# camillabelponer/dealii-slod

Hardware: AMD Instinct MI355X
Metric: SLOD patches/sec (basis built), 2D Poisson H=1/32 n_sub=8 oversampling 2 (higher is better)
Workload: dtype f64; 1 GPU; C2: 2D Poisson SLOD, H=1/32, n_sub=8, oversampling=2, D1e4 coefficient (contrast 10000), 1024 patches on rank 0 (ensemble of 1 realisations, contiguous patch blocks); patches_per_gpu=1024, parallelism=patch-sharded x1

## Files before the change

### dealii-slod_amd/csrc/slod_api.cpp

```cpp
#include "slod_host.h"

#include <algorithm>
#include <cmath>
#include <cstdio>
#include <cstdlib>
#include <cstring>
#include <string>
#include <vector>

namespace
{
  struct PatchGeom
  {
    int cx, cy, x0, y0, mx, my;
    int side_domain[4];
  };
}

std::string &slod_create_error()
{
  static thread_local std::string e;
  return e;
}

// ... 151 lines not shown
  {
    const slod_handle *h = p->h;
    SlodKernelArgs     a;
    std::memset(&a, 0, sizeof(a));
    a.desc        = (balanced && p->d_desc_bal ? p->d_desc_bal : p->d_desc) + first;
    a.coef0       = h->d_coef[0];
    a.coef1       = h->d_coef[1];
    a.coef_stride = (size_t)h->NE * h->NE * 4;
    a.NE          = h->NE;
    a.n_sub       = h->cfg.n_subdivisions;
    a.quirk       = h->cfg.projection_quirk;
#ifdef SLOD_ENABLE_DIAG
    if (const char *dg = std::getenv("SLOD_DIAG"))
      a.diag = std::atoi(dg);
#endif
    const double H = 1.0 / (double)h->N, hh = H / (double)h->cfg.n_subdivisions;
    a.scale     = hh * hh / 4.0;
    a.invH2     = 1.0 / (H * H);
    a.st        = p->ws_st;
    a.st_stride = p->st_stride;
    a.nn_max    = p->nn_max;
    a.vinv      = p->ws_v;
    a.v_stride  = p->v_stride;
    a.m_max     = p->m_max;
    a.L_max     = p->L_max;
    a.xs        = p->ws_x;
    a.zs        = p->ws_z ? p->ws_z : p->ws_x;
    a.x_stride  = p->x_stride;
    a.nc_max    = p->nc_max;
    a.ms        = p->ws_m;
    a.mt        = p->ws_m + p->chunk * (size_t)p->nc_max * p->nc_max;
    a.m_fused   = 0;
    a.m_tw      = 0;
    a.nb_buf    = p->nb_buf;
    a.nf_max    = p->nf_max;
    a.fuse_select = 0;
    a.fuse_assemble = 0;
    a.basis     = d_basis;
    a.premult   = d_premult;
    a.status    = p->d_status;
    a.pdiag     = p->d_pdiag;
    if (slot == 1)
      {
        a.st     = p->alt.ws_st;
        a.vinv   = p->alt.ws_v;
        a.xs     = p->alt.ws_x;
        a.zs     = p->alt.ws_z ? p->alt.ws_z : p->alt.ws_x;
        a.ms     = p->alt.ws_m;
        a.mt     = p->alt.ws_m + p->chunk * (size_t)p->nc_max * p->nc_max;
        a.status = p->alt.d_status;
      }
    return a;
  }
}

namespace
{
  hipError_t launch_range(slod_plan *p, size_t first, int cnt, double *d_basis, double *d_premult, hipStream_t st,
                          hipEvent_t *ev, bool balanced, int slot = 0)
  {
    const int      s = p->h->cfg.spacedim;
    SlodKernelArgs a = make_args(p, first, d_basis, d_premult, balanced, slot);
    hipError_t     e = ev ? hipEventRecord(ev[0], st) : hipSuccess;
    if (e == hipSuccess && !p->choice.fuse_assemble)
      e = slod_launch_assemble(s, a, cnt, st);
    if (e == hipSuccess && ev)
// ... 1013 lines not shown
```

### dealii-slod_amd/csrc/slod_device.h

```cpp
#ifndef SLOD_DEVICE_H
#define SLOD_DEVICE_H

#include <hip/hip_runtime.h>
#include <stddef.h>
#include <stdint.h>

struct SlodPatchDesc
{
  int32_t  ox, oy;
  int32_t  nx, ny;
  int32_t  mx, my;
  int32_t  ccx, ccy;
  int32_t  flags;
  int32_t  m, L;
  int32_t  n_c, n_b;
  int32_t  prob;
  uint32_t plan_index;
  uint64_t out_off;
};

__host__ __device__ inline size_t slod_mt_stride(int nc_max) { return (size_t)nc_max * nc_max + 1; }

enum : int32_t
{
// ... 16 lines not shown
  double  dinf;
  double  sigma_max, sigma_min;
};

struct SlodKernelArgs
{
  const SlodPatchDesc *desc;
  const double        *coef0;
  const double        *coef1;
  size_t               coef_stride;
  int32_t              NE;
  int32_t              n_sub;
  int32_t              quirk;
  int32_t              diag;
  int32_t              debug;
  double               scale;
  double               invH2;
  double *st;
  size_t  st_stride;
  int32_t nn_max;
  double *vinv;
  size_t  v_stride;
  int32_t m_max;
  int32_t L_max;
  int32_t nv;
  double *xs;
  double *zs;
  size_t  x_stride;
  int32_t nc_max;
  double *ms;
  int32_t m_fused;
  double *mt;
  int32_t m_tw;
  int32_t nb_buf;
  int32_t nf_max;
  int32_t fuse_select;
  int32_t fuse_assemble;
  double  *basis;
  double  *premult;
  int32_t *status;
  SlodPatchDiag *pdiag;
};

enum SlodSolverKind : int32_t
{
  SLOD_K_MF   = 1,
  SLOD_K_TW   = 2,
  SLOD_K_WS   = 3,
  SLOD_K_COOP = 4,
  SLOD_K_ND   = 5
};

struct SlodTuning
{
  int solver = 0;
  int fuse_select = 1, fuse_assemble = 1, fuse_m = -1;
  int twisted = -1;
  int balance = 1;
  int debug = 0;
};
struct SlodSolveChoice
{
  int    kind = 0;
  size_t lds  = 0;
  int    fuse_select = 0, fuse_assemble = 0, m_fused = 0, m_tw = 0, twisted = 0, debug = 0;
  int    v_line_pad = 0;
  size_t v_line_elems = 0;
  int    nv = 0;
  size_t v_patch_elems = 0;
};
SlodTuning slod_read_tuning();
bool       slod_choose_solver(int S, int n_sub, int m_max, int L_max, int nc_max, int nb_buf, int nf_max, size_t n_patches,
                              const SlodTuning &t, SlodSolveChoice *out);

hipError_t slod_launch_assemble(int S, const SlodKernelArgs &a, int n_patches, hipStream_t st);
hipError_t slod_launch_solve(int S, const SlodSolveChoice &c, SlodKernelArgs &a, int n_patches, hipStream_t st);
hipError_t slod_launch_solve_mf(int S, const SlodKernelArgs &a, int n_patches, size_t lds, hipStream_t st);
hipError_t slod_launch_solve_tw(int S, const SlodKernelArgs &a, int n_patches, size_t lds, hipStream_t st);
hipError_t slod_launch_solve_ws(int S, const SlodKernelArgs &a, int n_patches, size_t lds, hipStream_t st);
hipError_t slod_launch_solve_coop(int S, int twisted, const SlodKernelArgs &a, int n_patches, hipStream_t st);
hipError_t slod_launch_solve_nd(const SlodKernelArgs &a, int n_patches, size_t lds, hipStream_t st);
int        slod_solve_nd_cell(int S, int n_sub, int m_max, int L_max);
size_t     slod_solve_nd_scratch(int nv, int m_max, int L_max, int nc_max);
size_t     slod_solve_nd_lds_bytes(int nv, int m_max, int nc_max);
hipError_t slod_launch_select(int S, const SlodKernelArgs &a, int n_patches, int nb_max,
                              int nf_max, hipStream_t st);
size_t     slod_solve_lds_bytes(int S, int m_max, int nc_max, int twisted);
size_t     slod_solve_ws_lds_bytes(int S, int m_max, int nc_max);
size_t     slod_solve_tw_lds_bytes(int S, int m_max, int nc_max, bool with_m = false);
size_t     slod_solve_mf_lds_bytes(int S, int m_max, int nc_max);
int        slod_solve_ws_tile(int m_max);
int        slod_solve_mf_tiles(int S, int m_max);
size_t     slod_select_lds_bytes(int S, int nb_max, int nc_max, int nf_max);

#endif
```

### dealii-slod_amd/csrc/slod_dispatch.cpp

```cpp
#include "slod_device.h"

#include <algorithm>
#include <cstdlib>
#include <cstring>

SlodTuning slod_read_tuning()
{
  SlodTuning t;
  if (const char *sel = getenv("SLOD_SOLVE"))
    t.solver = !strcmp(sel, "mf") ? SLOD_K_MF : !strcmp(sel, "tw") ? SLOD_K_TW : !strcmp(sel, "ws") ? SLOD_K_WS :
               !strcmp(sel, "coop") ? SLOD_K_COOP : !strcmp(sel, "nd") ? SLOD_K_ND : 0;
  if (const char *e = getenv("SLOD_FUSE_SELECT"))
    t.fuse_select = atoi(e) ? 1 : 0;
  if (const char *e = getenv("SLOD_FUSE_ASSEMBLE"))
    t.fuse_assemble = atoi(e) ? 1 : 0;
  if (const char *e = getenv("SLOD_FUSE_M"))
    t.fuse_m = atoi(e) ? 1 : 0;
  if (const char *e = getenv("SLOD_TWISTED"))
    t.twisted = atoi(e) ? 1 : 0;
  if (const char *e = getenv("SLOD_BALANCE"))
    t.balance = atoi(e) ? 1 : 0;
  if (const char *e = getenv("SLOD_DEBUG"))
    t.debug = atoi(e) ? 1 : 0;
  return t;
}

bool slod_choose_solver(int S, int n_sub, int m_max, int L_max, int nc_max, int nb_buf, int nf_max, size_t n_patches,
                        const SlodTuning &t_in, SlodSolveChoice *out)
{
  const size_t    lds_max = 160 * 1024;
  SlodSolveChoice c;
  const int       nd_nv = slod_solve_nd_cell(S, n_sub, m_max, L_max);
  SlodTuning      t     = t_in;
  if (t.solver == SLOD_K_ND && nd_nv == 0)
    t.solver = 0;
  c.debug = t.debug;
  const int  wt = slod_solve_ws_tile(m_max);
  const bool ws_fits = wt > 0 && wt >= 2 * S - 1;
  const auto want = [&](int k) { return t.solver == 0 || t.solver == k; };
  const size_t lds_sel = slod_select_lds_bytes(S, nb_buf, nc_max, nf_max);
  const bool   mf_fits = slod_solve_mf_tiles(S, m_max) > 0 && slod_solve_mf_lds_bytes(S, m_max, nc_max) <= lds_max;
  const bool   tw_fits = ws_fits && slod_solve_tw_lds_bytes(S, m_max, nc_max) <= lds_max;
  if (nd_nv > 0 && t.solver == SLOD_K_ND)
    {
      c.kind          = SLOD_K_ND;
      c.nv            = nd_nv;
      c.lds           = slod_solve_nd_lds_bytes(nd_nv, m_max, nc_max);
      c.v_patch_elems = slod_solve_nd_scratch(nd_nv, m_max, L_max, nc_max);
      c.fuse_assemble = t.fuse_assemble ? 1 : 0;
      c.fuse_select   = 0;
    }
  else if (mf_fits && (t.solver == SLOD_K_MF || (t.solver == 0 && !tw_fits && !ws_fits)))
    {
      c.kind          = SLOD_K_MF;
      c.lds           = slod_solve_mf_lds_bytes(S, m_max, nc_max);
      c.v_line_pad    = 16 * slod_solve_mf_tiles(S, m_max);
      c.v_line_elems  = (size_t)c.v_line_pad * c.v_line_pad;
      c.fuse_assemble = (S == 1 && t.fuse_assemble) ? 1 : 0;
      c.fuse_select   = (S == 1 && t.fuse_select && lds_sel <= lds_max) ? 1 : 0;
      if (c.fuse_select && lds_sel > c.lds)
        c.lds = lds_sel;
    }
  else if (want(SLOD_K_TW) && tw_fits)
    {
      c.kind          = SLOD_K_TW;
      c.lds           = slod_solve_tw_lds_bytes(S, m_max, nc_max);
      c.v_line_pad    = 8 * wt;
      c.v_line_elems  = (size_t)64 * wt * wt;
      c.fuse_assemble = (S == 1 && t.fuse_assemble) ? 1 : 0;
      c.fuse_select = (S == 1 && t.fuse_select && lds_sel <= 64 * 1024) ? 1 : 0;
      if (S == 1 && t.fuse_m != 0 && nc_max <= 32 && 8 * wt <= 48)
        {
          const size_t sel    = c.fuse_select ? lds_sel : 0;
          const size_t with_m = std::max(slod_solve_tw_lds_bytes(S, m_max, nc_max, true), sel);
          if (std::min<size_t>(4, lds_max / with_m) == std::min<size_t>(4, lds_max / std::max(c.lds, sel)))
            {
              c.m_tw = 1;
              c.lds  = slod_solve_tw_lds_bytes(S, m_max, nc_max, true);
            }
        }
      if (c.fuse_select && lds_sel > c.lds)
        c.lds = lds_sel;
    }
  else if ((want(SLOD_K_WS) || t.solver == SLOD_K_TW) && ws_fits &&
           slod_solve_ws_lds_bytes(S, m_max, nc_max) <= lds_max)
    {
      c.kind       = SLOD_K_WS;
      c.lds        = slod_solve_ws_lds_bytes(S, m_max, nc_max);
      c.v_line_pad = 8 * wt;
      c.v_line_elems = (size_t)c.v_line_pad * c.v_line_pad;
      c.m_fused = (t.fuse_m > 0 && nc_max * nc_max <= 192 * 4) ? 1 : 0;
    }
  else if (t.solver == 0 || t.solver == SLOD_K_COOP || !ws_fits)
    {
      int tw = t.twisted >= 0 ? t.twisted : (n_patches < 3 * 256 ? 1 : 0);
      if (slod_solve_lds_bytes(S, m_max, nc_max, tw) > lds_max)
        tw = 0;
      if (slod_solve_lds_bytes(S, m_max, nc_max, tw) > lds_max || (m_max + 15) / 16 > 7)
        return false;
      c.kind       = SLOD_K_COOP;
      c.twisted    = tw;
      c.lds        = slod_solve_lds_bytes(S, m_max, nc_max, tw);
      c.v_line_pad = m_max;
      c.v_line_elems = (size_t)m_max * m_max;
    }
  else
    return false;
  if (!c.fuse_select && lds_sel > lds_max)
    return false;
  *out = c;
  return true;
}

hipError_t slod_launch_solve(int S, const SlodSolveChoice &c, SlodKernelArgs &a, int n_patches, hipStream_t st)
{
  a.m_fused       = c.m_fused;
  a.m_tw          = c.m_tw;
  a.fuse_select   = c.fuse_select;
  a.fuse_assemble = c.fuse_assemble;
  a.debug         = c.debug;
  switch (c.kind)
    {
      case SLOD_K_MF:
        return slod_launch_solve_mf(S, a, n_patches, c.lds, st);
      case SLOD_K_TW:
        return slod_launch_solve_tw(S, a, n_patches, c.lds, st);
      case SLOD_K_WS:
        return slod_launch_solve_ws(S, a, n_patches, c.lds, st);
      case SLOD_K_COOP:
        return slod_launch_solve_coop(S, c.twisted, a, n_patches, st);
      case SLOD_K_ND:
        a.nv = c.nv;
        return slod_launch_solve_nd(a, n_patches, c.lds, st);
      default:
        return hipErrorInvalidValue;
    }
}
```

### dealii-slod_amd/csrc/slod_solve_tw.hip

```cpp
#include <type_traits>
#include "slod_assemble.hip.h"
#include "slod_select.hip.h"

namespace
{
  template <int T, int S>
  __global__ __launch_bounds__(256, ws_min_waves(T)) void k_solve_tw(const SlodKernelArgs A)
  {
    extern __shared__ __attribute__((aligned(16))) double smem[];
    const SlodPatchDesc d = A.desc[blockIdx.x];
    constexpr int       W = 2 * S - 1, BW = 2 * W + 1, MP = 8 * T;
    constexpr int       BWP = BW + 1, BROWS = MP + 2 * W, bsz = (BROWS * BWP + 1) & ~1;
    const int           tid = threadIdx.x, wave = __builtin_amdgcn_readfirstlane(tid >> 6);
    int                 lane = tid & 63;
    const int           chain = wave & 1;
    const bool          is_gj = wave < 2;
    const int           m = d.m, L = d.L, nc = d.n_c, n = A.n_sub;
    const int           mm = A.m_max, ncs = (A.nc_max + 1) & ~1, ncg = A.nc_max;
    const bool          tr  = (d.flags & SLOD_F_TRANSPOSED) != 0;
    const int           npx = d.nx + 1;
    const int           chsz = MP * ncs + MP + 6 * bsz;

    double *cb   = smem + chain * chsz;
    double *Rb   = cb;
    double *rowb = Rb + MP * ncs;
    double *Tf   = rowb + MP;
    double *Tn0  = Tf + bsz;
    double *Tn1  = Tn0 + bsz;
    double *Bc0  = Tn1 + bsz;
    double *Bc1  = Bc0 + bsz;
    auto    Bbuf = [&](double *base, int stp) { return base + ((stp + 3) % 3) * bsz; };
    double *ocb  = smem + (1 - chain) * chsz;
    int    *colk = reinterpret_cast<int *>(smem + 2 * chsz);
    int *perm = colk + 2 * A.nc_max + chain * 3 * A.nc_max, *inv = perm + A.nc_max, *act = inv + A.nc_max;
    int *operm = colk + 2 * A.nc_max + (1 - chain) * 3 * A.nc_max, *oinv = operm + A.nc_max, *oact = oinv + A.nc_max;
    (void)operm;
    double *mtile = smem + 2 * chsz + 4 * A.nc_max;
    double *mfull = smem + chsz;
    bool    mfuse = false;
    auto nafin = [&](int ch) {
      const int *ac = colk + 2 * A.nc_max + ch * 3 * A.nc_max + 2 * A.nc_max;
      const int  nl = ch == 0 ? L / 2 : L - 1 - L / 2;
      int        na = 0;
      for (int k = 0; k < nc; ++k)
        na += ac[k] <= nl - 1 ? 1 : 0;
      return na;
    };

    const double *st    = A.st + (size_t)blockIdx.x * A.st_stride;
    double       *vg    = A.vinv + (size_t)blockIdx.x * A.v_stride;
    double       *xg    = A.xs + (size_t)blockIdx.x * A.x_stride;
    double       *zg    = A.zs + (size_t)blockIdx.x * A.x_stride;
    const size_t  vline = (size_t)64 * T * T, xline = (size_t)mm * ncg;
    auto load_A = [&](const double *vl, int ti, double (&dst)[MP / 4]) __attribute__((always_inline)) {
      const int     row = min(16 * ti + (lane & 15), MP - 1);
      const int     rt = row / T, rr = row - rt * T, kq = lane >> 4;
      const double *base = vl + (rt * 8 + kq) * (T * T) + rr * T;
#pragma unroll
      for (int g = 0; g < 2; ++g)
#pragma unroll
        for (int kr = 0; kr < T; ++kr)
          dst[g * T + kr] = base[g * 4 * T * T + kr];
    };
    auto brow = [&](int kk) { return T * ((lane >> 4) + 4 * (kk / T)) + kk % T; };

    const int mid = L / 2;
    double4_t pm[3] = {{0.0, 0.0, 0.0, 0.0}, {0.0, 0.0, 0.0, 0.0}, {0.0, 0.0, 0.0, 0.0}};
    auto mid_tile = [&](int ti, bool with_m) __attribute__((always_inline)) {
      const double *vl = vg + (size_t)mid * vline;
      double       *xl = xg + (size_t)mid * xline;
      const int     tiles_j = (nc + 15) >> 4;
// ... 85 lines not shown
            }
          if (wave == nw - 1)
            turn(true);
        }
      __syncthreads();
    };
    const int n0 = mid, n1 = L - 1 - mid, nstp = n0 > n1 ? n0 : n1;
    const int nmy = chain == 0 ? n0 : n1;
    const int dl  = chain == 0 ? 1 : -1;
    auto      line_of = [&](int c, int t) { return c == 0 ? t : L - 1 - t; };

    if ((SLOD_DG(A, (1 << 20))) && tid == 0)
      {
        A.ms[(size_t)blockIdx.x * A.nc_max * A.nc_max] = (double)wall_clock64();
        if (A.nc_max * A.nc_max >= 16)
          {
            A.ms[(size_t)blockIdx.x * A.nc_max * A.nc_max + 12] = (double)__builtin_amdgcn_s_getreg((31 << 11) | 4);
            A.ms[(size_t)blockIdx.x * A.nc_max * A.nc_max + 13] = (double)__builtin_amdgcn_s_getreg((31 << 11) | 20);
          }
      }
    if ((SLOD_DG(A, (1 << 20))) && lane == 0 && A.nc_max * A.nc_max >= 24)
      A.ms[(size_t)blockIdx.x * A.nc_max * A.nc_max + 20 + wave] = (double)__builtin_amdgcn_s_getreg((31 << 11) | 4);
    auto tstamp = [&](int k) {
      if ((SLOD_DG(A, (1 << 20))) && tid == 0 && A.nc_max * A.nc_max >= 48)
        A.ms[(size_t)blockIdx.x * A.nc_max * A.nc_max + 32 + k] = (double)wall_clock64();
    };
    tstamp(0);
    if (S == 1 && A.fuse_assemble)
      {
        for (int node = tid; node < npx * (d.ny + 1); node += 256)
          assemble_node<S>(A, d, blockIdx.x, node);
        __syncthreads();
      }
    for (int idx = tid; idx < 2 * chsz; idx += 256)
      smem[idx] = 0.0;
    if (A.m_tw)
      for (int idx = tid; idx < 2 * 256; idx += 256)
        mtile[idx] = 0.0;
    for (int c = tid; c < nc; c += 256)
      {
        int kx, ky;
        cell_of_col(d, c / S, kx, ky);
        colk[c]            = kx;
        colk[A.nc_max + c] = ky;
      }
    __syncthreads();
    {
      auto first_step = [&](int ch, int c) {
        const int kq = tr ? colk[c] : colk[A.nc_max + c];
        const int a  = ch == 0 ? kq * n - 1 : L - (kq + 1) * n;
        return a > 0 ? a : 0;
      };
      for (int idx = tid; idx < 2 * nc; idx += 256)
        {
          const int ch = idx / nc, c = idx - ch * nc, a = first_step(ch, c);
          int       rank = 0;
          for (int c2 = 0; c2 < nc; ++c2)
            {
              const int a2 = first_step(ch, c2);
              rank += (a2 < a || (a2 == a && c2 < c)) ? 1 : 0;
            }
          int *pp = colk + 2 * A.nc_max + ch * 3 * A.nc_max;
          pp[rank]                = c;
          pp[A.nc_max + c]        = rank;
          pp[2 * A.nc_max + rank] = a;
        }
    }
    auto put_bands = [&](int line, double *Tdst, bool with_T, double *Bdst, int t0, int nt) __attribute__((always_inline)) {
      for (int idx = t0; idx < m * BW; idx += nt)
        {
          const int i = idx / BW, oi = idx - i * BW, o = oi - W;
          if (Tdst)
            Tdst[(i + W) * BWP + oi] = with_T ? coupling<S>(st, A.nn_max, npx, tr, m, line, i, 0, o) : 0.0;
          if (Bdst)
            Bdst[(i + W) * BWP + oi] = coupling<S>(st, A.nn_max, npx, tr, m, line, i, dl, o);
        }
    };
    auto put_step = [&](int stp, int t0, int nt) __attribute__((always_inline)) {
      if (stp >= nmy)
        return;
      put_bands(line_of(chain, stp + 1), (stp & 1) ? Tn1 : Tn0, !(chain == 1 && stp + 1 == nmy), nullptr, t0, nt);
      put_bands(line_of(chain, stp), nullptr, true, Bbuf(Bc0, stp), t0, nt);
    };
    {
      const int t0 = (wave >> 1) * 64 + lane;
      put_bands(line_of(chain, 0), Tf, true, nullptr, t0, 128);
      put_step(0, t0, 128);
      put_step(1, t0, 128);
    }
    __syncthreads();
    tstamp(1);
    mfuse = S == 1 && A.m_tw && (MP + 15) / 16 <= 3 && nc <= 32 &&
                 nc * nc <= MP * ncs + MP + 3 * bsz && !(SLOD_DG(A, 8));
    int na_end[2] = {0, 0};
    if (mfuse)
      {
        na_end[0] = __builtin_amdgcn_readfirstlane(nafin(0));
        na_end[1] = __builtin_amdgcn_readfirstlane(nafin(1));
        mfuse     = na_end[0] <= 16 && na_end[1] <= 16;
      }
    if (A.m_tw && tid == 0)
      A.mt[(size_t)blockIdx.x * slod_mt_stride(A.nc_max) + (size_t)A.nc_max * A.nc_max] = mfuse ? 1.0 : 0.0;

    if (is_gj)
      {
        __builtin_amdgcn_s_setprio(3);
        int    gy = lane >> 3, gx = lane & 7;
        double a[T][T];
        auto dpp_from_prev = [](double x) {
          const int lo = __builtin_amdgcn_update_dpp(0, __double2loint(x), 0x111, 0xf, 0xf, true);
          const int hi = __builtin_amdgcn_update_dpp(0, __double2hiint(x), 0x111, 0xf, 0xf, true);
          return __hiloint2double(hi, lo);
        };
        auto dpp_from_next = [](double x) {
          const int lo = __builtin_amdgcn_update_dpp(0, __double2loint(x), 0x101, 0xf, 0xf, true);
// ... 202 lines not shown
          for (int ta = 0; ta < T; ++ta)
#pragma unroll
            for (int tb = 0; tb < T; ++tb)
              tp[ta * T + tb] = sign * a[ta][tb];
        };
#pragma unroll
        for (int ta = 0; ta < T; ++ta)
#pragma unroll
          for (int tb = 0; tb < T; ++tb)
            {
              const int      i = T * gy + ta, j = T * gx + tb;
              const unsigned oi = (unsigned)(j - i + W);
              const double   v  = Tf[(i + W) * BWP + (oi < (unsigned)BW ? oi : (unsigned)BW)];
              a[ta][tb]         = (chain == 1 && nmy == 0) ? 0.0 : v;
            }
        double acc_t[4] = {0.0, 0.0, 0.0, 0.0};
        for (int t = 0; t < nstp; ++t)
          {
            const bool active = t < nmy;
            asm volatile("" : "+v"(lane));
            gy = lane >> 3;
            gx = lane & 7;
            const long long c0 = (SLOD_DG(A, (1 << 20))) ? wall_clock64() : 0;
            long long       c1 = c0, c2 = c0;
            if (active)
              {
                sweep();
                c1 = (SLOD_DG(A, (1 << 20))) ? wall_clock64() : 0;
                if (!(SLOD_DG(A, 32768)))
                  store_tile(vg + (size_t)line_of(chain, t) * vline, -1.0);
                if (SLOD_DG(A, (1 << 20)))
                  acc_t[3] += (double)(wall_clock64() - c1);
                if (!(SLOD_DG(A, 16384)))
                  next_S((t & 1) ? Tn1 : Tn0, Bbuf(Bc0, t));
                c2 = (SLOD_DG(A, (1 << 20))) ? wall_clock64() : 0;
              }
            __syncthreads();
            if (SLOD_DG(A, (1 << 20)))
              {
                const long long c3 = wall_clock64();
                acc_t[0] += (double)(c1 - c0);
                acc_t[1] += (double)(c2 - c1);
                acc_t[2] += (double)(c3 - c2);
              }
          }
        if ((SLOD_DG(A, (1 << 20))) && tid == 0 && A.nc_max * A.nc_max >= 48)
          {
            for (int k = 0; k < 4; ++k)
              A.ms[(size_t)blockIdx.x * A.nc_max * A.nc_max + 40 + k] = acc_t[k];
            if (A.nc_max * A.nc_max >= 52)
              for (int k = 0; k < 2; ++k)
                A.ms[(size_t)blockIdx.x * A.nc_max * A.nc_max + 48 + k] = acc_p[k];
          }
        tstamp(2);
        if (chain == 1)
          store_tile(vg + (size_t)mid * vline, 1.0);
        __syncthreads();
        if (chain == 0)
          {
            const double *w1 = vg + (size_t)mid * vline + (gy * 8 + gx) * (T * T);
#pragma unroll
            for (int ta = 0; ta < T; ++ta)
#pragma unroll
              for (int tb = 0; tb < T; ++tb)
                a[ta][tb] += w1[ta * T + tb];
            sweep();
            store_tile(vg + (size_t)mid * vline, -1.0);
// ... 162 lines not shown
                    {
                      acc0 = __builtin_amdgcn_mfma_f64_16x16x4f64(av[kk], bq[0][kk], acc0, 0, 0, 0);
                      if (two)
                        acc1 = __builtin_amdgcn_mfma_f64_16x16x4f64(av[kk], bq[1][kk], acc1, 0, 0, 0);
                    }
#pragma unroll
                  for (int r = 0; r < 4; ++r)
                    {
                      const int row = 16 * ti + (lane >> 4) + 4 * r, col = lane & 15;
                      if (row < m && col < ncols)
                        {
                          xl[row * ncols + col] = acc0[r];
                          Rb[row * ncs + col]   = acc0[r];
                        }
                      if (two && row < m && col + 16 < ncols)
                        {
                          xl[row * ncols + col + 16] = acc1[r];
                          Rb[row * ncs + col + 16]   = acc1[r];
                        }
                    }
                  if (ti + 1 < TI)
                    {
#pragma unroll
                      for (int kk = 0; kk < MP / 4; ++kk)
                        av[kk] = an[kk];
                    }
                }
            }
          __builtin_amdgcn_fence(__ATOMIC_RELEASE, "wavefront");
          __builtin_amdgcn_wave_barrier();
          if (mfuse)
            {
              __builtin_amdgcn_fence(__ATOMIC_ACQUIRE, "wavefront");
              double   *mtc = mtile + chain * 256 + (lane >> 4) * 16 + (lane & 15);
              double4_t macc;
#pragma unroll
              for (int r = 0; r < 4; ++r)
                macc[r] = mtc[64 * r];
#pragma unroll
              for (int kk = 0; kk < MP / 4; ++kk)
                macc = __builtin_amdgcn_mfma_f64_16x16x4f64(bq[0][kk], bp[brow(kk) * ncs], macc, 0, 0, 0);
#pragma unroll
              for (int r = 0; r < 4; ++r)
                mtc[64 * r] = macc[r];
              __builtin_amdgcn_fence(__ATOMIC_RELEASE, "wavefront");
              __builtin_amdgcn_wave_barrier();
            }
        };
        constexpr int NBQ = (MP * BW + 63) / 64;
        double        tq[NBQ], bq_[NBQ];
        auto fetch_step = [&](int stp) __attribute__((always_inline)) {
          const bool on = stp < nmy;
          const int  lT = line_of(chain, stp + 1), lB = line_of(chain, stp);
          const bool with_T = !(chain == 1 && stp + 1 == nmy);
#pragma unroll
          for (int q = 0; q < NBQ; ++q)
            {
              const int  idx = lane + 64 * q, i = idx / BW, oi = idx - i * BW, o = oi - W, j = i + o;
              const int  pi = i / S, ci = i - pi * S, pj = j / S, cj = j - pj * S, dp = pj - pi;
              const bool ok = on && idx < m * BW && j >= 0 && j < m && dp >= -1 && dp <= 1;
              const int ixT = tr ? lT + 1 : pi + 1, iyT = tr ? pi + 1 : lT + 1;
              const int ixB = tr ? lB + 1 : pi + 1, iyB = tr ? pi + 1 : lB + 1;
              const int dirT = (tr ? dp : 0) * 3 + (tr ? 0 : dp) + 4;
              const int dirB = ((tr ? dp : dl) + 1) * 3 + (tr ? dl : dp) + 1;
              const double vT = st[ok ? (size_t)((dirT * S + ci) * S + cj) * A.nn_max + ixT + iyT * npx : 0];
              const double vB = st[ok ? (size_t)((dirB * S + ci) * S + cj) * A.nn_max + ixB + iyB * npx : 0];
              tq[q]  = (ok && with_T) ? vT : 0.0;
              bq_[q] = ok ? vB : 0.0;
            }
        };
        auto store_step = [&](int stp) __attribute__((always_inline)) {
          if (stp >= nmy)
            return;
          double *Tdst = (stp & 1) ? Tn1 : Tn0, *Bdst = Bbuf(Bc0, stp);
#pragma unroll
          for (int q = 0; q < NBQ; ++q)
            {
              const int idx = lane + 64 * q, i = idx / BW, oi = idx - i * BW;
              if (idx < m * BW)
                {
                  Tdst[(i + W) * BWP + oi] = tq[q];
                  Bdst[(i + W) * BWP + oi] = bq_[q];
                }
            }
        };
        double acc_h[4] = {0.0, 0.0, 0.0, 0.0};
        int  na = 0;
        bool z_in_lds = false;
        auto fwd_step = [&](int tl) __attribute__((always_inline)) {
          const int na_prev = na;
          while (na < nc && act[na] <= tl)
            ++na;
          const int line = line_of(chain, tl);
          const long long b0 = (SLOD_DG(A, (1 << 20))) ? wall_clock64() : 0;
          const bool keep = TI <= 3 && na <= 32 && !(SLOD_DG(A, 8));
          if (keep)
            {
              double av[MP / 4];
              load_A(vg + (size_t)line * vline, 0, av);
              build_R(line, Bbuf(Bc0, tl - 1), tl > 0 ? zg + (size_t)line_of(chain, tl - 1) * xline : nullptr, na_prev,
                      true, false, na, perm, nullptr, act, tl - 1, z_in_lds);
              __builtin_amdgcn_fence(__ATOMIC_RELEASE, "wavefront");
              __builtin_amdgcn_wave_barrier();
              if (SLOD_DG(A, (1 << 20)))
                acc_h[3] += (double)(wall_clock64() - b0);
              gemm_Z_keep(line, na, zg + (size_t)line * xline, av);
              z_in_lds = true;
              return;
            }
          build_R(line, Bbuf(Bc0, tl - 1), tl > 0 ? zg + (size_t)line_of(chain, tl - 1) * xline : nullptr, na_prev, true,
                  false, na, perm, nullptr, act, tl - 1, false);
          __builtin_amdgcn_fence(__ATOMIC_RELEASE, "wavefront");
          __builtin_amdgcn_wave_barrier();
          if (SLOD_DG(A, (1 << 20)))
            acc_h[3] += (double)(wall_clock64() - b0);
          gemm_Z(line, na, zg + (size_t)line * xline, na);
          z_in_lds = false;
        };
        for (int t = 0; t < nstp; ++t)
          {
            asm volatile("" : "+v"(lane));
            const long long c0 = (SLOD_DG(A, (1 << 20))) ? wall_clock64() : 0;
            if (t > 0 && !(SLOD_DG(A, 32)))
              fetch_step(t + 1);
            if (t > 0 && t - 1 < nmy)
              fwd_step(t - 1);
            const long long c1 = (SLOD_DG(A, (1 << 20))) ? wall_clock64() : 0;
            if (t > 0 && !(SLOD_DG(A, 32)))
              store_step(t + 1);
            const long long c2 = (SLOD_DG(A, (1 << 20))) ? wall_clock64() : 0;
            __syncthreads();
            if (SLOD_DG(A, (1 << 20)))
              {
                const long long c3 = wall_clock64();
                acc_h[0] += (double)(c1 - c0);
                acc_h[1] += (double)(c2 - c1);
                acc_h[2] += (double)(c3 - c2);
              }
          }
        if ((SLOD_DG(A, (1 << 20))) && tid == 128 && A.nc_max * A.nc_max >= 48)
          for (int k = 0; k < 4; ++k)
            A.ms[(size_t)blockIdx.x * A.nc_max * A.nc_max + 44 + k] = acc_h[k];
        if (nmy == nstp && nmy > 0)
          fwd_step(nstp - 1);
        __syncthreads();
        if (chain == 0)
          {
            const double *B0 = Bbuf(Bc0, n0 - 1);
            double       *ob = ocb + MP * ncs + MP + 3 * bsz;
            const double *B1 = Bbuf(ob, n1 - 1);
            int na0 = 0, na1 = 0;
            while (na0 < nc && act[na0] <= n0 - 1)
              ++na0;
            while (na1 < nc && oact[na1] <= n1 - 1)
              ++na1;
            build_R(mid, B0, n0 > 0 ? zg + (size_t)(mid - 1) * xline : nullptr, na0, true, false, nc, nullptr, inv, act,
                    n0 - 1, false);
            __builtin_amdgcn_wave_barrier();
            if (n1 > 0)
              build_R(mid, B1, zg + (size_t)(mid + 1) * xline, na1, false, true, nc, nullptr, oinv, oact, n1 - 1, false);
            __builtin_amdgcn_fence(__ATOMIC_RELEASE, "wavefront");
            __builtin_amdgcn_wave_barrier();
          }
        else if (mfuse)
          {
            const int na0 = na_end[0], na1 = na_end[1];
            for (int idx = lane; idx < nc * nc; idx += 64)
              {
                const int a = idx / nc, b = idx - a * nc, lo = min(a, b), hi = max(a, b);
                double    v = 0.0;
#pragma unroll
                for (int ch = 0; ch < 2; ++ch)
                  {
                    const int *ci = colk + 2 * A.nc_max + ch * 3 * A.nc_max + A.nc_max;
                    const int  i0 = ci[lo], j0 = ci[hi];
                    if (i0 < (ch ? na1 : na0) && j0 < (ch ? na1 : na0))
                      v += mtile[ch * 256 + i0 * 16 + j0];
                  }
                mfull[idx] = v;
              }
          }
        __syncthreads();
        mid_phase();
      }

    tstamp(3);
    {
      const int t128 = (wave >> 1) * 64 + lane, w2 = wave >> 1;
      const int tiles_i = (m + 15) >> 4, tiles_j = (nc + 15) >> 4;
      constexpr int NBV = (MP * BW + 127) / 128;
      double        bv[NBV];
      auto fetch_B = [&](int line) __attribute__((always_inline)) {
#pragma unroll
        for (int q = 0; q < NBV; ++q)
          {
            const int idx = t128 + 128 * q, i = idx / BW, o = idx - i * BW - W;
            bv[q] = (idx < m * BW) ? coupling<S>(st, A.nn_max, npx, tr, m, line, i, dl, o) : 0.0;
          }
      };
      auto store_B = [&](double *Bdst) __attribute__((always_inline)) {
#pragma unroll
        for (int q = 0; q < NBV; ++q)
          {
            const int idx = t128 + 128 * q, i = idx / BW, oi = idx - i * BW;
            if (idx < m * BW)
              Bdst[(i + W) * BWP + oi] = bv[q];
          }
      };
      const int tstart = (SLOD_DG(A, 16)) ? -1 : nstp - 1;
      if (tstart >= 0 && tstart < nmy)
        {
          fetch_B(line_of(chain, tstart));
          store_B((tstart & 1) ? Bc1 : Bc0);
        }
      else if (nmy > 0 && tstart >= 0)
        {
          fetch_B(line_of(chain, nmy - 1));
          store_B(((nmy - 1) & 1) ? Bc1 : Bc0);
        }
      int nab = nc;
      constexpr int TIB   = (MP + 15) / 16;
      const bool    keepb = TIB <= 3 && nc <= 32 && !(SLOD_DG(A, 64));
      if (keepb)
        for (int idx = t128; idx < m * nc; idx += 128)
          {
            const int i = idx / nc, c = idx - i * nc;
            Rb[i * ncs + c] = xg[(size_t)mid * xline + i * ncg + c];
          }
      auto backward = [&](auto KEEP) __attribute__((always_inline)) {
      constexpr bool keep_x = decltype(KEEP)::value;
      for (int t = tstart; t >= 0; --t)
        {
          while (nab > 0 && act[nab - 1] > t)
            --nab;
          const bool    active = t < nmy;
          const int     line = line_of(chain, t), prev = line_of(chain, t + 1);
          const double *Bn = (t & 1) ? Bc1 : Bc0;
          asm volatile("" : "+v"(lane));
          __syncthreads();
          if (active && t > 0)
            fetch_B(line_of(chain, t - 1));
          if constexpr (keep_x)
            {
              const double *vl = vg + (size_t)line * vline;
              double       *xl = xg + (size_t)line * xline;
              const int     g = lane >> 3, cq = lane & 7;
              const int     colw = 16 * w2 + (lane & 15);
              const bool    gemm = active && 16 * w2 < nc;
              constexpr int NPRE = 1;
              double        av[NPRE][MP / 4], zl[NPRE][4];
              const double *zrow = zg + (size_t)line * xline;
              const int     zc   = colw < nc ? inv[colw] : nc;
              const bool    zok  = zc < nab;
              auto          load_Z = [&](int ti, double (&dst)[4]) __attribute__((always_inline)) {
#pragma unroll
                for (int r = 0; r < 4; ++r)
                  {
                    const int    row = 16 * ti + (lane >> 4) + 4 * r;
                    const bool   ok  = row < m && zok;
                    const double z   = zrow[ok ? row * nab + zc : 0];
                    dst[r]           = ok ? z : 0.0;
                  }
              };
              if (gemm)
                {
#pragma unroll
                  for (int ti = 0; ti < NPRE; ++ti)
                    if (ti < tiles_i)
                      {
                        load_A(vl, ti, av[ti]);
                        load_Z(ti, zl[ti]);
                      }
                }
              double y[2][T];
              if (active)
                {
#pragma unroll
                  for (int k = 0; k < 2; ++k)
                    {
                      const int c = cq + 8 * (2 * w2 + k);
                      double    win[T + 2 * W];
#pragma unroll
                      for (int e = 0; e < T + 2 * W; ++e)
                        {
                          const int    pr  = T * g + e - W;
                          const bool   inb = c < nc && pr >= 0 && pr < m;
                          const double x   = Rb[(inb ? pr : 0) * ncs + (inb ? c : 0)];
                          win[e]           = inb ? x : 0.0;
                        }
#pragma unroll
                      for (int ta = 0; ta < T; ++ta)
                        {
                          double v = 0.0;
#pragma unroll
                          for (int o = 0; o < BW; ++o)
                            v = fma(Bn[(T * g + ta + W) * BWP + o], win[ta + o], v);
                          y[k][ta] = v;
                        }
                    }
                }
              __builtin_amdgcn_fence(__ATOMIC_RELEASE, "wavefront");
              __builtin_amdgcn_wave_barrier();
              __builtin_amdgcn_fence(__ATOMIC_ACQUIRE, "wavefront");
              if (active)
                {
#pragma unroll
                  for (int k = 0; k < 2; ++k)
                    {
                      const int c = cq + 8 * (2 * w2 + k);
#pragma unroll
                      for (int ta = 0; ta < T; ++ta)
                        if (c < nc && T * g + ta < m)
                          Rb[(T * g + ta) * ncs + c] = y[k][ta];
                    }
                }
              __builtin_amdgcn_fence(__ATOMIC_RELEASE, "wavefront");
              __builtin_amdgcn_wave_barrier();
              __builtin_amdgcn_fence(__ATOMIC_ACQUIRE, "wavefront");
              double bq[MP / 4];
              if (gemm)
                {
#pragma unroll
                  for (int kk = 0; kk < MP / 4; ++kk)
                    bq[kk] = Rb[brow(kk) * ncs + colw];
                }
              __builtin_amdgcn_fence(__ATOMIC_RELEASE, "wavefront");
              __builtin_amdgcn_wave_barrier();
              __builtin_amdgcn_fence(__ATOMIC_ACQUIRE, "wavefront");
              if (gemm)
                {
#pragma unroll
                  for (int ti = 0; ti < TIB; ++ti)
                    if (ti < tiles_i)
                      {
                        double4_t acc = {0.0, 0.0, 0.0, 0.0};
                        double    zt[4];
                        if (ti < NPRE)
                          {
#pragma unroll
                            for (int kk = 0; kk < MP / 4; ++kk)
                              acc = __builtin_amdgcn_mfma_f64_16x16x4f64(av[ti < NPRE ? ti : 0][kk], bq[kk], acc, 0, 0, 0);
#pragma unroll
                            for (int r = 0; r < 4; ++r)
                              zt[r] = zl[ti < NPRE ? ti : 0][r];
                          }
                        else
                          {
                            double al[MP / 4];
                            load_A(vl, ti, al);
                            load_Z(ti, zt);
#pragma unroll
                            for (int kk = 0; kk < MP / 4; ++kk)
                              acc = __builtin_amdgcn_mfma_f64_16x16x4f64(al[kk], bq[kk], acc, 0, 0, 0);
                          }
#pragma unroll
                        for (int r = 0; r < 4; ++r)
                          {
                            const int row = 16 * ti + (lane >> 4) + 4 * r;
                            if (row < m && colw < nc)
                              {
                                const double x       = zt[r] - acc[r];
                                xl[row * ncg + colw] = x;
                                Rb[row * ncs + colw] = x;
                              }
                          }
                      }
                }
              if (active && t > 0)
                store_B(((t - 1) & 1) ? Bc1 : Bc0);
              continue;
            }
          if (active)
            {
              const double *xp = xg + (size_t)prev * xline;
              const int     qr = t128 >> 5, i_lo = (qr * m) >> 2, i_hi = ((qr + 1) * m) >> 2;
              for (int r = t128 & 31; r < nc; r += 32)
                {
                  double win[BW];
#pragma unroll
                  for (int e = 0; e < BW; ++e)
                    {
                      const int p = i_lo + e - W;
                      win[e]      = (p >= 0 && p < m) ? xp[p * ncg + r] : 0.0;
                    }
                  for (int i = i_lo; i < i_hi; ++i)
                    {
                      const int    pn    = i + 1 + W;
                      const double xnext = (pn < m) ? xp[pn * ncg + r] : 0.0;
                      double       v     = 0.0;
#pragma unroll
                      for (int o = 0; o < BW; ++o)
                        v = fma(Bn[(i + W) * BWP + o], win[o], v);
                      Rb[i * ncs + r] = v;
#pragma unroll
                      for (int e = 0; e + 1 < BW; ++e)
                        win[e] = win[e + 1];
                      win[BW - 1] = xnext;
                    }
                }
            }
          __syncthreads();
          if (active)
// ... 4 lines not shown
                {
                  const int ti = tt / tiles_j, tj = tt - ti * tiles_j;
                  const int col = 16 * tj + (lane & 15);
                  const double *zrow = zg + (size_t)line * xline;
                  const int     zc   = col < nc ? inv[col] : nc;
                  const bool    zok  = zc < nab;
                  double        zl[4];
#pragma unroll
                  for (int r = 0; r < 4; ++r)
                    {
                      const int row = 16 * ti + (lane >> 4) + 4 * r;
                      zl[r]         = (row < m && zok) ? zrow[row * nab + zc] : 0.0;
                    }
                  double4_t     acc = {0.0, 0.0, 0.0, 0.0};
                  const double *bp  = Rb + col;
                  double        av[MP / 4];
                  load_A(vl, ti, av);
#pragma unroll
                  for (int kk = 0; kk < MP / 4; ++kk)
                    acc = __builtin_amdgcn_mfma_f64_16x16x4f64(av[kk], bp[brow(kk) * ncs], acc, 0, 0, 0);
#pragma unroll
                  for (int r = 0; r < 4; ++r)
                    {
                      const int row = 16 * ti + (lane >> 4) + 4 * r;
                      if (row < m && col < nc)
                        xl[row * ncg + col] = zl[r] - acc[r];
                    }
                }
              if (t > 0)
                store_B(((t - 1) & 1) ? Bc1 : Bc0);
            }
        }
      };
      if (keepb)
        backward(std::true_type{});
      else
        backward(std::false_type{});
    }
    const bool stamp = (SLOD_DG(A, (1 << 20))) && tid == 0;
    if (stamp)
      A.ms[(size_t)blockIdx.x * A.nc_max * A.nc_max + 1] = (double)wall_clock64();
    if (S == 1 && A.fuse_select)
      {
        __syncthreads();
        select_patch<S>(A, A.nb_buf, A.nf_max, blockIdx.x, smem,
                        mfuse ? A.mt + (size_t)blockIdx.x * slod_mt_stride(A.nc_max) : nullptr);
        if (stamp)
          A.ms[(size_t)blockIdx.x * A.nc_max * A.nc_max + 2] = (double)wall_clock64();
      }
  }

}

size_t slod_solve_tw_lds_bytes(int S, int m_max, int nc_max, bool with_m)
{
  const int    T = slod_solve_ws_tile(m_max), W = 2 * S - 1, BW = 2 * W + 1, MP = 8 * T;
  const int    ncs = (nc_max + 1) & ~1, bsz = ((MP + 2 * W) * (BW + 1) + 1) & ~1;
  (void)m_max;
  const size_t chsz  = (size_t)MP * ncs + MP + 6 * (size_t)bsz;
  const size_t mtile = with_m ? 2 * 256 * sizeof(double) : 0;
  return ((2 * chsz * sizeof(double) + 8 * (size_t)nc_max * sizeof(int) + mtile) + 15) & ~(size_t)15;
}

template <int T, int S>
static hipError_t launch_tw_TS(const SlodKernelArgs &a, int n_patches, size_t lds, hipStream_t st)
{
  const void *fn = reinterpret_cast<const void *>(k_solve_tw<T, S>);
  hipError_t  e  = hipFuncSetAttribute(fn, hipFuncAttributeMaxDynamicSharedMemorySize, (int)lds);
  if (e != hipSuccess)
    return e;
  if (a.debug)
    {
      int nb = 0;
      (void)hipOccupancyMaxActiveBlocksPerMultiprocessor(&nb, fn, 256, lds);
      fprintf(stderr, "[slod] k_solve_tw<%d,%d>: %d patches, lds %zu B, occupancy %d blocks/CU, M in the sweeps %d\n", T,
              S, n_patches, lds, nb, a.m_tw);
    }
  hipLaunchKernelGGL((k_solve_tw<T, S>), dim3(n_patches), dim3(256), lds, st, a);
  return hipGetLastError();
}

template <int S>
static hipError_t launch_tw_S(const SlodKernelArgs &a, int n_patches, size_t lds, hipStream_t st)
{
  switch (slod_solve_ws_tile(a.m_max))
    {
      case 2:
        return launch_tw_TS<2, S>(a, n_patches, lds, st);
      case 3:
        return launch_tw_TS<3, S>(a, n_patches, lds, st);
      case 4:
        return launch_tw_TS<4, S>(a, n_patches, lds, st);
      case 5:
        return launch_tw_TS<5, S>(a, n_patches, lds, st);
      case 6:
        return launch_tw_TS<6, S>(a, n_patches, lds, st);
      case 8:
        return launch_tw_TS<8, S>(a, n_patches, lds, st);
      case 10:
        return launch_tw_TS<10, S>(a, n_patches, lds, st);
      case 12:
        return launch_tw_TS<12, S>(a, n_patches, lds, st);
      case 14:
        return launch_tw_TS<14, S>(a, n_patches, lds, st);
      default:
        return hipErrorInvalidValue;
    }
}

// ... 5 lines not shown
```

Before: 1.045 million patches/s.

## Stream backward-sweep V tiles into LDS via global_load_lds DMA in twisted solver

Adds an optional mode, on by default under SLOD_BW_DMA, for the twisted block-tridiagonal solver with S=1. In this mode the backward sweep copies the later V (inverse block) tiles of each line into LDS with global_load_lds direct-to-LDS transfers and reads the MFMA A operands from LDS instead of global memory. To fit this, the LDS layout is rearranged so the two chains share and reuse the idle buffer space, with the third B buffer relocated and a mode that is enabled only when blocks-per-CU occupancy stays the same. It also adds timing instrumentation behind the diag flag. The cost is a more complex LDS aliasing scheme and an extra block barrier per line, which risks layout bugs between chains.

Measured after the change: 877,200 patches/s, median of 2. -16.0%, worse.

```diff
diff --git a/dealii-slod_amd/csrc/slod_api.cpp b/dealii-slod_amd/csrc/slod_api.cpp
--- a/dealii-slod_amd/csrc/slod_api.cpp
+++ b/dealii-slod_amd/csrc/slod_api.cpp
@@ -207,6 +207,7 @@
     a.mt        = p->ws_m + p->chunk * (size_t)p->nc_max * p->nc_max;
     a.m_fused   = 0;
     a.m_tw      = 0;
+    a.bw_dma    = 0;
     a.nb_buf    = p->nb_buf;
     a.nf_max    = p->nf_max;
     a.fuse_select = 0;
diff --git a/dealii-slod_amd/csrc/slod_device.h b/dealii-slod_amd/csrc/slod_device.h
--- a/dealii-slod_amd/csrc/slod_device.h
+++ b/dealii-slod_amd/csrc/slod_device.h
@@ -72,6 +72,7 @@
   int32_t m_fused;
   double *mt;
   int32_t m_tw;
+  int32_t bw_dma;
   int32_t nb_buf;
   int32_t nf_max;
   int32_t fuse_select;
@@ -95,6 +96,7 @@
 {
   int solver = 0;
   int fuse_select = 1, fuse_assemble = 1, fuse_m = -1;
+  int bw_dma = 1;
   int twisted = -1;
   int balance = 1;
   int debug = 0;
@@ -103,7 +105,7 @@
 {
   int    kind = 0;
   size_t lds  = 0;
-  int    fuse_select = 0, fuse_assemble = 0, m_fused = 0, m_tw = 0, twisted = 0, debug = 0;
+  int    fuse_select = 0, fuse_assemble = 0, m_fused = 0, m_tw = 0, bw_dma = 0, twisted = 0, debug = 0;
   int    v_line_pad = 0;
   size_t v_line_elems = 0;
   int    nv = 0;
@@ -127,7 +129,7 @@
                               int nf_max, hipStream_t st);
 size_t     slod_solve_lds_bytes(int S, int m_max, int nc_max, int twisted);
 size_t     slod_solve_ws_lds_bytes(int S, int m_max, int nc_max);
-size_t     slod_solve_tw_lds_bytes(int S, int m_max, int nc_max, bool with_m = false);
+size_t     slod_solve_tw_lds_bytes(int S, int m_max, int nc_max, bool with_m = false, bool dma = false);
 size_t     slod_solve_mf_lds_bytes(int S, int m_max, int nc_max);
 int        slod_solve_ws_tile(int m_max);
 int        slod_solve_mf_tiles(int S, int m_max);
diff --git a/dealii-slod_amd/csrc/slod_dispatch.cpp b/dealii-slod_amd/csrc/slod_dispatch.cpp
--- a/dealii-slod_amd/csrc/slod_dispatch.cpp
+++ b/dealii-slod_amd/csrc/slod_dispatch.cpp
@@ -16,6 +16,8 @@
     t.fuse_assemble = atoi(e) ? 1 : 0;
   if (const char *e = getenv("SLOD_FUSE_M"))
     t.fuse_m = atoi(e) ? 1 : 0;
+  if (const char *e = getenv("SLOD_BW_DMA"))
+    t.bw_dma = atoi(e) ? 1 : 0;
   if (const char *e = getenv("SLOD_TWISTED"))
     t.twisted = atoi(e) ? 1 : 0;
   if (const char *e = getenv("SLOD_BALANCE"))
@@ -79,6 +81,16 @@
               c.lds  = slod_solve_tw_lds_bytes(S, m_max, nc_max, true);
             }
         }
+      if (S == 1 && t.bw_dma && nc_max <= 32 && 8 * wt > 16 && 8 * wt <= 48)
+        {
+          const size_t sel  = c.fuse_select ? lds_sel : 0;
+          const size_t with = std::max(slod_solve_tw_lds_bytes(S, m_max, nc_max, c.m_tw != 0, true), sel);
+          if (std::min<size_t>(4, lds_max / with) == std::min<size_t>(4, lds_max / std::max(c.lds, sel)))
+            {
+              c.bw_dma = 1;
+              c.lds    = slod_solve_tw_lds_bytes(S, m_max, nc_max, c.m_tw != 0, true);
+            }
+        }
       if (c.fuse_select && lds_sel > c.lds)
         c.lds = lds_sel;
     }
@@ -116,6 +128,7 @@
 {
   a.m_fused       = c.m_fused;
   a.m_tw          = c.m_tw;
+  a.bw_dma        = c.bw_dma;
   a.fuse_select   = c.fuse_select;
   a.fuse_assemble = c.fuse_assemble;
   a.debug         = c.debug;
diff --git a/dealii-slod_amd/csrc/slod_solve_tw.hip b/dealii-slod_amd/csrc/slod_solve_tw.hip
--- a/dealii-slod_amd/csrc/slod_solve_tw.hip
+++ b/dealii-slod_amd/csrc/slod_solve_tw.hip
@@ -4,6 +4,24 @@
 
 namespace
 {
+  struct TwLds
+  {
+    int bsz, used, idle, vsz, ints, total;
+    __host__ __device__ static constexpr int v_first(int T) { return (16 / T) * 8 * T * T; }
+    __host__ __device__ TwLds(int T, int S, int nc_max, bool with_m, bool dma)
+    {
+      const int W = 2 * S - 1, BW = 2 * W + 1, MP = 8 * T, ncs = (nc_max + 1) & ~1;
+      bsz   = ((MP + 2 * W) * (BW + 1) + 1) & ~1;
+      used  = MP * ncs + 2 * bsz;
+      idle  = MP + 4 * bsz;
+      vsz   = idle + (with_m ? 256 : 0);
+      if (dma && vsz < 64 * T * T - v_first(T))
+        vsz = 64 * T * T - v_first(T);
+      ints  = (4 * nc_max + 1) & ~1;
+      total = 2 * (used + vsz) + ints;
+    }
+  };
+
   template <int T, int S>
   __global__ __launch_bounds__(256, ws_min_waves(T)) void k_solve_tw(const SlodKernelArgs A)
   {
@@ -19,24 +37,28 @@
     const int           mm = A.m_max, ncs = (A.nc_max + 1) & ~1, ncg = A.nc_max;
     const bool          tr  = (d.flags & SLOD_F_TRANSPOSED) != 0;
     const int           npx = d.nx + 1;
-    const int           chsz = MP * ncs + MP + 6 * bsz;
+    const TwLds         lay(T, S, A.nc_max, A.m_tw != 0, A.bw_dma != 0);
 
-    double *cb   = smem + chain * chsz;
-    double *Rb   = cb;
-    double *rowb = Rb + MP * ncs;
-    double *Tf   = rowb + MP;
-    double *Tn0  = Tf + bsz;
-    double *Tn1  = Tn0 + bsz;
-    double *Bc0  = Tn1 + bsz;
+    double *vs0  = smem + lay.used + lay.ints, *vs1 = vs0 + lay.vsz;
+    double *Rb   = chain == 0 ? smem : vs1 + lay.vsz;
+    double *Bc0  = Rb + MP * ncs;
     double *Bc1  = Bc0 + bsz;
-    auto    Bbuf = [&](double *base, int stp) { return base + ((stp + 3) % 3) * bsz; };
-    double *ocb  = smem + (1 - chain) * chsz;
-    int    *colk = reinterpret_cast<int *>(smem + 2 * chsz);
+    double *rowb = chain == 0 ? vs0 : Rb - MP;
+    double *Tf   = chain == 0 ? rowb + MP : rowb - bsz;
+    double *Tn0  = chain == 0 ? Tf + bsz : Tf - bsz;
+    double *Tn1  = chain == 0 ? Tn0 + bsz : Tn0 - bsz;
+    double *Bc2  = chain == 0 ? Tn1 + bsz : Tn1 - bsz;
+    double *Vs   = chain == 0 ? vs0 : vs1;
+    auto    Bbuf = [&](double *b01, double *b2, int stp) {
+      const int k = (stp + 3) % 3;
+      return k == 2 ? b2 : b01 + k * bsz;
+    };
+    int    *colk = reinterpret_cast<int *>(smem + lay.used);
     int *perm = colk + 2 * A.nc_max + chain * 3 * A.nc_max, *inv = perm + A.nc_max, *act = inv + A.nc_max;
     int *operm = colk + 2 * A.nc_max + (1 - chain) * 3 * A.nc_max, *oinv = operm + A.nc_max, *oact = oinv + A.nc_max;
     (void)operm;
-    double *mtile = smem + 2 * chsz + 4 * A.nc_max;
-    double *mfull = smem + chsz;
+    double *mtile0 = vs0 + lay.idle, *mtile1 = vs1 + lay.vsz - lay.idle - 256;
+    double *mfull  = vs1 + lay.vsz - (MP + 3 * bsz);
     bool    mfuse = false;
     auto nafin = [&](int ch) {
       const int *ac = colk + 2 * A.nc_max + ch * 3 * A.nc_max + 2 * A.nc_max;
@@ -188,11 +210,10 @@
           assemble_node<S>(A, d, blockIdx.x, node);
         __syncthreads();
       }
-    for (int idx = tid; idx < 2 * chsz; idx += 256)
+    for (int idx = tid; idx < lay.used; idx += 256)
       smem[idx] = 0.0;
-    if (A.m_tw)
-      for (int idx = tid; idx < 2 * 256; idx += 256)
-        mtile[idx] = 0.0;
+    for (int idx = tid; idx < 2 * lay.vsz + lay.used; idx += 256)
+      vs0[idx] = 0.0;
     for (int c = tid; c < nc; c += 256)
       {
         int kx, ky;
@@ -236,7 +257,7 @@
       if (stp >= nmy)
         return;
       put_bands(line_of(chain, stp + 1), (stp & 1) ? Tn1 : Tn0, !(chain == 1 && stp + 1 == nmy), nullptr, t0, nt);
-      put_bands(line_of(chain, stp), nullptr, true, Bbuf(Bc0, stp), t0, nt);
+      put_bands(line_of(chain, stp), nullptr, true, Bbuf(Bc0, Bc2, stp), t0, nt);
     };
     {
       const int t0 = (wave >> 1) * 64 + lane;
@@ -505,7 +526,7 @@
                 if (SLOD_DG(A, (1 << 20)))
                   acc_t[3] += (double)(wall_clock64() - c1);
                 if (!(SLOD_DG(A, 16384)))
-                  next_S((t & 1) ? Tn1 : Tn0, Bbuf(Bc0, t));
+                  next_S((t & 1) ? Tn1 : Tn0, Bbuf(Bc0, Bc2, t));
                 c2 = (SLOD_DG(A, (1 << 20))) ? wall_clock64() : 0;
               }
             __syncthreads();
@@ -734,7 +755,7 @@
           if (mfuse)
             {
               __builtin_amdgcn_fence(__ATOMIC_ACQUIRE, "wavefront");
-              double   *mtc = mtile + chain * 256 + (lane >> 4) * 16 + (lane & 15);
+              double   *mtc = (chain == 0 ? mtile0 : mtile1) + (lane >> 4) * 16 + (lane & 15);
               double4_t macc;
 #pragma unroll
               for (int r = 0; r < 4; ++r)
@@ -774,7 +795,7 @@
         auto store_step = [&](int stp) __attribute__((always_inline)) {
           if (stp >= nmy)
             return;
-          double *Tdst = (stp & 1) ? Tn1 : Tn0, *Bdst = Bbuf(Bc0, stp);
+          double *Tdst = (stp & 1) ? Tn1 : Tn0, *Bdst = Bbuf(Bc0, Bc2, stp);
 #pragma unroll
           for (int q = 0; q < NBQ; ++q)
             {
@@ -800,7 +821,7 @@
             {
               double av[MP / 4];
               load_A(vg + (size_t)line * vline, 0, av);
-              build_R(line, Bbuf(Bc0, tl - 1), tl > 0 ? zg + (size_t)line_of(chain, tl - 1) * xline : nullptr, na_prev,
+              build_R(line, Bbuf(Bc0, Bc2, tl - 1), tl > 0 ? zg + (size_t)line_of(chain, tl - 1) * xline : nullptr, na_prev,
                       true, false, na, perm, nullptr, act, tl - 1, z_in_lds);
               __builtin_amdgcn_fence(__ATOMIC_RELEASE, "wavefront");
               __builtin_amdgcn_wave_barrier();
@@ -810,7 +831,7 @@
               z_in_lds = true;
               return;
             }
-          build_R(line, Bbuf(Bc0, tl - 1), tl > 0 ? zg + (size_t)line_of(chain, tl - 1) * xline : nullptr, na_prev, true,
+          build_R(line, Bbuf(Bc0, Bc2, tl - 1), tl > 0 ? zg + (size_t)line_of(chain, tl - 1) * xline : nullptr, na_prev, true,
                   false, na, perm, nullptr, act, tl - 1, false);
           __builtin_amdgcn_fence(__ATOMIC_RELEASE, "wavefront");
           __builtin_amdgcn_wave_barrier();
@@ -848,9 +869,9 @@
         __syncthreads();
         if (chain == 0)
           {
-            const double *B0 = Bbuf(Bc0, n0 - 1);
-            double       *ob = ocb + MP * ncs + MP + 3 * bsz;
-            const double *B1 = Bbuf(ob, n1 - 1);
+            const double *B0 = Bbuf(Bc0, Bc2, n0 - 1);
+            double       *ob = vs1 + lay.vsz + MP * ncs;
+            const double *B1 = Bbuf(ob, vs1 + lay.vsz - (MP + 4 * bsz), n1 - 1);
             int na0 = 0, na1 = 0;
             while (na0 < nc && act[na0] <= n0 - 1)
               ++na0;
@@ -877,7 +898,7 @@
                     const int *ci = colk + 2 * A.nc_max + ch * 3 * A.nc_max + A.nc_max;
                     const int  i0 = ci[lo], j0 = ci[hi];
                     if (i0 < (ch ? na1 : na0) && j0 < (ch ? na1 : na0))
-                      v += mtile[ch * 256 + i0 * 16 + j0];
+                      v += (ch ? mtile1 : mtile0)[i0 * 16 + j0];
                   }
                 mfull[idx] = v;
               }
@@ -929,8 +950,18 @@
             const int i = idx / nc, c = idx - i * nc;
             Rb[i * ncs + c] = xg[(size_t)mid * xline + i * ncg + c];
           }
-      auto backward = [&](auto KEEP) __attribute__((always_inline)) {
-      constexpr bool keep_x = decltype(KEEP)::value;
+      double    acc_b[8] = {0.0, 0.0, 0.0, 0.0, 0.0, 0.0, 0.0, 0.0};
+      long long bc = 0;
+      auto      bstamp = [&](int k) __attribute__((always_inline)) {
+        if (SLOD_DG(A, (1 << 20)))
+          {
+            const long long now = wall_clock64();
+            acc_b[k] += (double)(now - bc);
+            bc = now;
+          }
+      };
+      auto backward = [&](auto MODE) __attribute__((always_inline)) {
+      constexpr bool keep_x = decltype(MODE)::value >= 1, dma = decltype(MODE)::value == 2;
       for (int t = tstart; t >= 0; --t)
         {
           while (nab > 0 && act[nab - 1] > t)
@@ -939,7 +970,10 @@
           const int     line = line_of(chain, t), prev = line_of(chain, t + 1);
           const double *Bn = (t & 1) ? Bc1 : Bc0;
           asm volatile("" : "+v"(lane));
+          if (SLOD_DG(A, (1 << 20)))
+            bc = wall_clock64();
           __syncthreads();
+          bstamp(0);
           if (active && t > 0)
             fetch_B(line_of(chain, t - 1));
           if constexpr (keep_x)
@@ -950,7 +984,8 @@
               const int     colw = 16 * w2 + (lane & 15);
               const bool    gemm = active && 16 * w2 < nc;
               constexpr int NPRE = 1;
-              double        av[NPRE][MP / 4], zl[NPRE][4];
+              constexpr int NZ   = dma ? TIB : NPRE;
+              double        av[NPRE][MP / 4], zl[NZ][4];
               const double *zrow = zg + (size_t)line * xline;
               const int     zc   = colw < nc ? inv[colw] : nc;
               const bool    zok  = zc < nab;
@@ -973,6 +1008,29 @@
                         load_A(vl, ti, av[ti]);
                         load_Z(ti, zl[ti]);
                       }
+                  if constexpr (dma)
+                    {
+#pragma unroll
+                      for (int ti = NPRE; ti < TIB; ++ti)
+                        load_Z(ti, zl[ti]);
+                    }
+                }
+              if constexpr (dma)
+                {
+                  if (active && tiles_i > 1)
+                    {
+                      constexpr int nchunk = (MP * MP - TwLds::v_first(T)) / 2;
+                      const double *src    = vl + TwLds::v_first(T);
+#pragma unroll
+                      for (int q = 0; 128 * q < nchunk; ++q)
+                        {
+                          const int c0 = 64 * (2 * q + w2);
+                          if (c0 + lane < nchunk)
+                            __builtin_amdgcn_global_load_lds(
+                              (const __attribute__((address_space(1))) void *)(src + 2 * (c0 + lane)),
+                              (__attribute__((address_space(3))) void *)(Vs + 2 * c0), 16, 0, 0);
+                        }
+                    }
                 }
               double y[2][T];
               if (active)
@@ -1025,19 +1083,45 @@
 #pragma unroll
                   for (int kk = 0; kk < MP / 4; ++kk)
                     bq[kk] = Rb[brow(kk) * ncs + colw];
-                }
+                  if (SLOD_DG(A, (1 << 20)))
+                    asm volatile("" : "+v"(bq[MP / 4 - 1]));
+                }
+              bstamp(1);
               __builtin_amdgcn_fence(__ATOMIC_RELEASE, "wavefront");
               __builtin_amdgcn_wave_barrier();
               __builtin_amdgcn_fence(__ATOMIC_ACQUIRE, "wavefront");
-              if (gemm)
-                {
-#pragma unroll
-                  for (int ti = 0; ti < TIB; ++ti)
-                    if (ti < tiles_i)
+#pragma unroll
+              for (int ti = 0; ti < TIB; ++ti)
+                {
+                  if (dma && ti == NPRE)
+                    {
+                      __builtin_amdgcn_s_waitcnt(0x0f70);
+                      __syncthreads();
+                      bstamp(3);
+                    }
+                  if (gemm && ti < tiles_i)
                       {
                         double4_t acc = {0.0, 0.0, 0.0, 0.0};
                         double    zt[4];
-                        if (ti < NPRE)
+                        if (dma && ti >= NPRE)
+                          {
+                            const int     row = min(16 * ti + (lane & 15), MP - 1);
+                            const int     rt = row / T, rr = row - rt * T, kq = lane >> 4;
+                            const double *base = Vs + ((rt * 8 + kq) * (T * T) + rr * T - TwLds::v_first(T));
+                            double        al[MP / 4];
+#pragma unroll
+                            for (int g2 = 0; g2 < 2; ++g2)
+#pragma unroll
+                              for (int kr = 0; kr < T; ++kr)
+                                al[g2 * T + kr] = base[g2 * 4 * T * T + kr];
+#pragma unroll
+                            for (int kk = 0; kk < MP / 4; ++kk)
+                              acc = __builtin_amdgcn_mfma_f64_16x16x4f64(al[kk], bq[kk], acc, 0, 0, 0);
+#pragma unroll
+                            for (int r = 0; r < 4; ++r)
+                              zt[r] = zl[ti < NZ ? ti : 0][r];
+                          }
+                        else if (ti < NPRE)
                           {
 #pragma unroll
                             for (int kk = 0; kk < MP / 4; ++kk)
@@ -1051,6 +1135,11 @@
                             double al[MP / 4];
                             load_A(vl, ti, al);
                             load_Z(ti, zt);
+                            if (!dma && (SLOD_DG(A, (1 << 20))))
+                              {
+                                asm volatile("" : "+v"(zt[3]));
+                                bstamp(1 + 2 * ti);
+                              }
 #pragma unroll
                             for (int kk = 0; kk < MP / 4; ++kk)
                               acc = __builtin_amdgcn_mfma_f64_16x16x4f64(al[kk], bq[kk], acc, 0, 0, 0);
@@ -1066,10 +1155,16 @@
                                 Rb[row * ncs + colw] = x;
                               }
                           }
+                        if (SLOD_DG(A, (1 << 20)))
+                          {
+                            asm volatile("" : "+v"(acc[3]));
+                            bstamp(2 + 2 * ti);
+                          }
                       }
                 }
               if (active && t > 0)
                 store_B(((t - 1) & 1) ? Bc1 : Bc0);
+              bstamp(7);
               continue;
             }
           if (active)
@@ -1140,10 +1235,15 @@
             }
         }
       };
-      if (keepb)
-        backward(std::true_type{});
+      if (keepb && S == 1 && TIB >= 2 && A.bw_dma)
+        backward(std::integral_constant<int, (S == 1 && TIB >= 2 && TIB <= 3) ? 2 : 1>{});
+      else if (keepb)
+        backward(std::integral_constant<int, 1>{});
       else
-        backward(std::false_type{});
+        backward(std::integral_constant<int, 0>{});
+      if ((SLOD_DG(A, (1 << 20))) && (tid == 0 || tid == 128) && A.nc_max * A.nc_max >= 72)
+        for (int k = 0; k < 8; ++k)
+          A.ms[(size_t)blockIdx.x * A.nc_max * A.nc_max + 56 + 8 * w2 + k] = acc_b[k];
     }
     const bool stamp = (SLOD_DG(A, (1 << 20))) && tid == 0;
     if (stamp)
@@ -1160,14 +1260,10 @@
 
 }
 
-size_t slod_solve_tw_lds_bytes(int S, int m_max, int nc_max, bool with_m)
+size_t slod_solve_tw_lds_bytes(int S, int m_max, int nc_max, bool with_m, bool dma)
 {
-  const int    T = slod_solve_ws_tile(m_max), W = 2 * S - 1, BW = 2 * W + 1, MP = 8 * T;
-  const int    ncs = (nc_max + 1) & ~1, bsz = ((MP + 2 * W) * (BW + 1) + 1) & ~1;
-  (void)m_max;
-  const size_t chsz  = (size_t)MP * ncs + MP + 6 * (size_t)bsz;
-  const size_t mtile = with_m ? 2 * 256 * sizeof(double) : 0;
-  return ((2 * chsz * sizeof(double) + 8 * (size_t)nc_max * sizeof(int) + mtile) + 15) & ~(size_t)15;
+  const TwLds lay(slod_solve_ws_tile(m_max), S, nc_max, with_m, dma);
+  return (size_t)lay.total * sizeof(double);
 }
 
 template <int T, int S>
@@ -1181,8 +1277,8 @@
     {
       int nb = 0;
       (void)hipOccupancyMaxActiveBlocksPerMultiprocessor(&nb, fn, 256, lds);
-      fprintf(stderr, "[slod] k_solve_tw<%d,%d>: %d patches, lds %zu B, occupancy %d blocks/CU, M in the sweeps %d\n", T,
-              S, n_patches, lds, nb, a.m_tw);
+      fprintf(stderr, "[slod] k_solve_tw<%d,%d>: %d patches, lds %zu B, occupancy %d blocks/CU, M in the sweeps %d, backward V by LDS-DMA %d\n",
+              T, S, n_patches, lds, nb, a.m_tw, a.bw_dma);
     }
   hipLaunchKernelGGL((k_solve_tw<T, S>), dim3(n_patches), dim3(256), lds, st, a);
   return hipGetLastError();
```
